# zhangzhousuper/Radish_PT

Measured on AMD Instinct MI355X. Metric: Mrays/s, higher is better.
Workload: dtype f32

## Files before the change

### radish_pt_amd/api.py

```python
import ctypes as C
import os

import numpy as np

from . import hostlib
from . import layouts as L

_HERE = os.path.dirname(os.path.abspath(__file__))
HIP_LIB_PATH = os.environ.get("RADISH_HIP_LIB") or os.path.join(_HERE, "csrc", "libradish_hip.so")

RDH_PT_MEGAKERNEL, RDH_PT_WAVEFRONT, RDH_PT_SORT_MATERIAL, RDH_PT_COUNT, RDH_PT_PROFILE = 0, 1, 2, 4, 8
RDH_PT_PERSISTENT = 16
RDH_PT_NO_SCHEDULE = 32
RDH_PT_ONE_LANE_PER_PIXEL = 64
RDH_PT_MEGA_GBUFFER = RDH_PT_ONE_LANE_PER_PIXEL
RDH_PT_NO_DEFER = 128
RDH_PT_WG_PER_RAY = 256
RDH_PT_PARTITION_GBUFFER = 512
RDH_PT_RESTIR_FUSED = 1024
RDH_PT_WF_SUBFRAMES = 2048
RDH_PT_WF_SMALL_LISTS = 4096
RDH_PT_NO_PAIRS = 16384
RDH_PT_NO_PACKETS = 8192
RDH_PT_PAIRS = 32768
# ... 595 lines not shown
        self.rank, self.world = rank, world

    def comm_destroy(self):
        self.check(lib().rdh_comm_destroy(self.h))

    @staticmethod
    def comm_init_all(ctxs):
        n = len(ctxs)
        arr = (C.c_void_p * n)(*[c.h for c in ctxs])
        rc = lib().rdh_comm_init_all(arr, n)
        if rc != 0:
            ctxs[0].check(rc)
        for i, c in enumerate(ctxs):
            c.rank, c.world = i, n

    @staticmethod
    def path_trace_gathered_all(ctxs, direct_frames, indirect_frames, iter, looper, max_depth, flags=RDH_PT_PERSISTENT):
        n = len(ctxs)
        arr = (C.c_void_p * n)(*[c.h for c in ctxs])
        px = ctxs[0].width * ctxs[0].height * 3
        d = (C.c_void_p * n)(*[c._ptr(t, px, "path_trace_gathered_all: direct") for c, t in zip(ctxs, direct_frames)])
        i = (C.c_void_p * n)(*[c._ptr(t, px, "path_trace_gathered_all: indirect") for c, t in zip(ctxs, indirect_frames)])
        rc = lib().rdh_path_trace_gathered_all(arr, n, d, i, iter, looper, max_depth, flags)
        if rc != 0:
            msgs = [lib().rdh_last_error(c.h) for c in ctxs]
            raise RadishError(f"libradish_hip error {rc}: " + "; ".join(f"ctx {k}: {m.decode()}" for k, m in enumerate(msgs) if m))

    def allgather_tiles(self, packed, frame):
        shard = self.tiles_per_rank() * self.tile * self.tile * 3
        self.check(lib().rdh_allgather_tiles(self.h, self._ptr(packed, shard, "allgather_tiles: packed"),
                                             self._ptr(frame, self.width * self.height * 3, "allgather_tiles: frame")))

    def path_trace_gathered(self, direct_frame, indirect_frame, iter, looper, max_depth, flags=RDH_PT_PERSISTENT):
        n = self.width * self.height * 3
        self.check(lib().rdh_path_trace_gathered(self.h, self._ptr(direct_frame, n, "path_trace_gathered: direct"),
                                                 self._ptr(indirect_frame, n, "path_trace_gathered: indirect"), iter, looper,
                                                 max_depth, flags))

    def restir_exchange(self):
        self.check(lib().rdh_restir_exchange(self.h))

    def comm_set_overlap(self, enable):
        self.check(lib().rdh_comm_set_overlap(self.h, 1 if enable else 0))

    def comm_join(self):
        self.check(lib().rdh_comm_join(self.h))

    @staticmethod
    def _all_error(ctxs, rc):
        msgs = [lib().rdh_last_error(c.h) for c in ctxs]
        raise RadishError(f"libradish_hip error {rc}: " + "; ".join(f"ctx {k}: {m.decode()}" for k, m in enumerate(msgs) if m))

    @staticmethod
    def gbuffer_exchange_all(ctxs, gb_cs):
        n = len(ctxs)
        arr = (C.c_void_p * n)(*[c.h for c in ctxs])
        gbs = (GBufferC * n)(*gb_cs)
        rc = lib().rdh_gbuffer_exchange_all(arr, n, gbs)
        if rc != 0:
            Context._all_error(ctxs, rc)

    @staticmethod
    def restir_direct_gathered_all(ctxs, direct_frames, iter, looper, gb_cs, reuse_mask, ris_count=32, num_spatial=5, temporal_clamp=20,
                                   faithful_ris=1, flags=0):
        n = len(ctxs)
        arr = (C.c_void_p * n)(*[c.h for c in ctxs])
        px = ctxs[0].width * ctxs[0].height * 3
        d = (C.c_void_p * n)(*[c._ptr(t, px, "restir_direct_gathered_all") for c, t in zip(ctxs, direct_frames)])
        gbs = (GBufferC * n)(*gb_cs)
        p = RestirParamsC(reuse_mask, ris_count, num_spatial, temporal_clamp, faithful_ris)
        rc = lib().rdh_restir_direct_gathered_all(arr, n, d, iter, looper, gbs, C.byref(p), flags)
        if rc != 0:
            Context._all_error(ctxs, rc)

    def restir_direct_gathered(self, direct_frame, iter, looper, gb_c, reuse_mask, ris_count=32, num_spatial=5, temporal_clamp=20,
                               faithful_ris=1, flags=0):
        p = RestirParamsC(reuse_mask, ris_count, num_spatial, temporal_clamp, faithful_ris)
        self.check(lib().rdh_restir_direct_gathered(self.h, self._ptr(direct_frame, self.width * self.height * 3, "restir_direct_gathered"),
                                                    iter, looper, C.byref(gb_c), C.byref(p), flags))

    def gbuffer_exchange(self, gb_c):
        self.check(lib().rdh_gbuffer_exchange(self.h, C.byref(gb_c)))

    def restir_read(self, which):
        out = np.zeros(self.width * self.height, dtype=L.RESERVOIR_DTYPE)
        self.check(lib().rdh_restir_read(self.h, which, out.ctypes.data))
        return out

    def restir_read_scratch(self, which):
        nbytes = int(lib().rdh_restir_read_scratch(self.h, which, None, 0))
        if nbytes < 0:
            self.check(nbytes)
        out = np.zeros(nbytes // 4, np.int32 if which == 2 else np.float32)
        got = int(lib().rdh_restir_read_scratch(self.h, which, out.ctypes.data, nbytes))
        if got < 0:
            self.check(got)
        return out if which == 2 else out.reshape(-1, 6)

    def trace_closest(self, rays, hits, flags=RDH_PT_PERSISTENT):
        n = rays.numel() // 6
        self.check(lib().rdh_trace_closest(self.h, self._ptr(rays, 6 * n, "trace_closest: rays"), n,
                                           self._ptr(hits, 4 * n, "trace_closest: hits", _torch().int32), flags))

    def trace_occluded(self, segments, out, flags=RDH_PT_PERSISTENT):
        n = segments.numel() // 6
        self.check(lib().rdh_trace_occluded(self.h, self._ptr(segments, 6 * n, "trace_occluded: segments"), n,
                                            self._ptr(out, n, "trace_occluded: out", _torch().int32), flags))

    def dump_rays(self, looper, max_depth):
        torch = _torch()
        nc, na = C.c_int64(0), C.c_int64(0)
        self.check(lib().rdh_dump_rays(self.h, looper, max_depth, None, 0, None, 0, C.byref(nc), C.byref(na)))
        dev = torch.device("cuda", self.device)
        closest = torch.zeros(max(nc.value, 1), 6, device=dev)
        segs = torch.zeros(max(na.value, 1), 6, device=dev)
        n2, a2 = C.c_int64(0), C.c_int64(0)
        self.check(lib().rdh_dump_rays(self.h, looper, max_depth, closest.data_ptr(), nc.value, segs.data_ptr(), na.value,
                                       C.byref(n2), C.byref(a2)))
        assert (n2.value, a2.value) == (nc.value, na.value)
        return closest[:nc.value], segs[:na.value]

    def set_occupancy_share(self, share):
        self.check(lib().rdh_set_occupancy_share(self.h, share))

    def counters_reset(self):
        self.check(lib().rdh_counters_reset(self.h))

    def counters(self):
        c = CountersC()
        self.check(lib().rdh_counters_read(self.h, C.byref(c)))
        return c.as_dict()

    def synchronize(self):
        self.check(lib().rdh_synchronize(self.h))

    def profile_reset(self):
        self.check(lib().rdh_profile_reset(self.h))

    def profile_read(self):
        ms, n = C.c_double(0), C.c_int64(0)
        self.check(lib().rdh_profile_read(self.h, C.byref(ms), C.byref(n)))
        return ms.value, n.value

    def debug_persist_stamps(self):
        out = np.zeros((5, 4096), dtype=np.uint64)
        self.check(lib().rdh_debug_persist_stamps(self.h, out.ctypes.data))
        return out

    def debug_wf_stamps(self):
        fn = lib().rdh_debug_wf_stamps
        fn.argtypes, fn.restype = [C.c_void_p, C.c_void_p, C.c_int64, C.POINTER(C.c_int32), C.POINTER(C.c_int32)], C.c_int32
        stages, waves = C.c_int32(0), C.c_int32(0)
        self.check(fn(self.h, None, 0, C.byref(stages), C.byref(waves)))
        out = np.zeros((stages.value, waves.value, 3), dtype=np.uint64)
        self.check(fn(self.h, out.ctypes.data, out.size, C.byref(stages), C.byref(waves)))
        return out

    def debug_persist_phases(self):
        out = np.zeros(16, dtype=np.uint64)
        self.check(lib().rdh_debug_persist_phases(self.h, out.ctypes.data))
        return out

    def last_kernel_ms(self):
        ms = C.c_float(0)
        self.check(lib().rdh_last_kernel_ms(self.h, C.byref(ms)))
        return ms.value


class ReservoirReuse:
    NONE, Temporal, Spatial, TemporalSpatial = 0, 1, 2, 3


class Settings:
    traceDepth = 0
    useReservoir = True
    reservoirReuse = ReservoirReuse.Temporal
    accumulate = False
    ptFlags = RDH_PT_PERSISTENT
    restirNumSpatial = 5
    restirRISCount = 32
    restirTemporalClamp = 20
    restirFaithfulRIS = 1


class State:
    camChanged = True
    looper = 0
    scene = None


class DevScene:

    def __init__(self):
        self.ctx = None

    def create(self, scene_data, device=0):
        self.ctx = Context(device)
        self.ctx.upload_scene(scene_data)

    def destroy(self):
        if self.ctx:
            self.ctx.close()
            self.ctx = None


class Scene:

    def __init__(self, scene_data, camera, device=0):
        self.data = scene_data
        self.camera = camera
        self.devScene = DevScene()
        self.devScene.create(scene_data, device)

    def clear(self):
        self.devScene.destroy()


def _ctx():
    if State.scene is None or State.scene.devScene.ctx is None:
        raise RadishError("State.scene is not set")
    ctx = State.scene.devScene.ctx
    ctx.set_camera(State.scene.camera)
    return ctx


def _advance_looper():
    State.looper = (State.looper + 1) % SOBOL_SAMPLE_NUM


def pathTraceInit():
    _ctx().synchronize()


def pathTraceFree():
    pass


def pathTrace(directIllum, indirectIllum, iter):
    ctx = _ctx()
    ctx.path_trace(directIllum, indirectIllum, iter, State.looper, Settings.traceDepth, Settings.ptFlags)
    ctx.synchronize()
    _advance_looper()


def pathTraceSamples(directIllum, indirectIllum, iter, samples):
    ctx = _ctx()
    ctx.path_trace_samples(directIllum, indirectIllum, iter, State.looper, samples, Settings.traceDepth, Settings.ptFlags)
    ctx.synchronize()
    State.looper = (State.looper + samples) % SOBOL_SAMPLE_NUM


def pathTraceDirect(directIllum, iter):
    ctx = _ctx()
    ctx.path_trace_direct(directIllum, iter, State.looper, Settings.ptFlags & RDH_PT_COUNT)
    ctx.synchronize()
    _advance_looper()


class ToneMapping:
    NONE, Filmic, ACES = 0, 1, 2


def copyImageToPBO(devPBO, devImage, width, height, toneMapping=ToneMapping.NONE, scale=1.0):
    torch = _torch()
    n = width * height
    if devImage.dtype == torch.int32:
        kind = 3
    elif devImage.dtype == torch.float32:
        kind = {3 * n: 0, 2 * n: 1, n: 2}.get(devImage.numel())
    else:
        kind = None
    if kind is None or devPBO.numel() * devPBO.element_size() != 4 * n:
        raise RadishError("copyImageToPBO: image/PBO shape does not match width*height")
    _ctx().copy_image_to_pbo(devPBO, devImage, width, height, kind, toneMapping, scale)


def ReSTIRInit():
    _ctx().restir_init()


def ReSTIRFree():
    if State.scene is not None and State.scene.devScene.ctx is not None:
        State.scene.devScene.ctx.restir_free()


def ReSTIRDirect(directIllum, iter, gBuffer):
    ctx = _ctx()
    ctx.restir_direct(directIllum, iter, State.looper, gBuffer.c_struct(), Settings.reservoirReuse,
                      Settings.restirRISCount, Settings.restirNumSpatial, Settings.restirTemporalClamp,
                      Settings.restirFaithfulRIS, Settings.ptFlags & RDH_PT_COUNT)
    ctx.synchronize()
    _advance_looper()


class GBuffer:

    def __init__(self):
        self.width = self.height = 0
        self.frameIdx = 0
        self.lastCam = None

    def create(self, width, height, device=0):
        torch = _torch()
        n = width * height
        dev = torch.device("cuda", device)
        self.width, self.height = width, height
        self.albedo = torch.zeros(n, 3, dtype=torch.float32, device=dev)
# ... 135 lines not shown
```

### radish_pt_amd/csrc/device/kernels_wave.h

```cpp
#pragma once
#include "kernels_pt.h"
#include "wg_trace.h"

namespace rd {

constexpr int kWfLitCap = 8192;
constexpr int kWfLitShadow = 0x40000000;
constexpr int kMaxWaveDepth = 32;

struct alignas(128) WaveCounter {
    int v;
    int pad[31];
};
#ifndef RD_WF_TICKET_SHARDS
#define RD_WF_TICKET_SHARDS 8
#endif
constexpr int kTicketShards = RD_WF_TICKET_SHARDS;
struct WaveCounters {
    WaveCounter rayCount[kMaxWaveDepth + 2];
    WaveCounter shadowCount[kMaxWaveDepth + 2];
    WaveCounter litCount[kMaxWaveDepth + 2];
    WaveCounter traceHead[kMaxWaveDepth + 2];
    WaveCounter shadeHead[kMaxWaveDepth + 2][4];
    WaveCounter traceTicket[kMaxWaveDepth + 2][kTicketShards];
    WaveCounter shadeTicket[kMaxWaveDepth + 2][kTicketShards];
};

struct WaveWorkspace {
    float4 *ro[2];
    float4 *rd[2];
    float4 *thr[2];
    float4 *prevPos[2];
    float4 *accD;
    float4 *accI;
    float4 *nee[2];
    float4 *sht[2];
    uint2 *rng[2];
    int4 *hit;
    int *rayq[2];
    int *shadowq;
    int *litq[2];
    int litCap;
    int *treeOvf;
    int treeOvfDepth;
#ifdef RD_WF_STAMPS
    unsigned long long *stamps;
    int stampWaves;
#endif
    WaveCounters *ctr;
};

constexpr unsigned kWfNeeNone = 2u;
RD_DEV float wfNeeTag(int home, unsigned kind) { return __uint_as_float(((unsigned)home << 2) | kind); }
RD_DEV void wfAddNee(const WaveWorkspace &w, float4 n) {
    const unsigned tag = __float_as_uint(n.w), kind = tag & 3u;
    if (kind == kWfNeeNone) return;
    float4 *acc = (kind == 0u ? w.accD : w.accI) + (tag >> 2);
    const float4 a = *acc;
    *acc = make_float4(a.x + n.x, a.y + n.y, a.z + n.z, 0.f);
}

RD_DEV Ray wfSlotRay(const WaveWorkspace &w, int set, int p, bool shadow, float &limit) {
    if (shadow) {
        const float4 x = w.prevPos[set][p], y = w.sht[set][p];
        return shadowRay(mk3(x.x, x.y, x.z), mk3(y.x, y.y, y.z), limit);
    }
    const float4 o = w.ro[set][p], d = w.rd[set][p];
    limit = 3.402823466e+38f;
    return Ray{mk3(o.x, o.y, o.z), mk3(d.x, d.y, d.z)};
}

struct WaveSlotPath {
    const WaveWorkspace &w;
    const int rs, p;
    const int wr, q;
    int home;
    const bool delta;
    RD_DEV v3 throughput() {
        const float4 t = w.thr[rs][p];
        home = __float_as_int(t.w);
        return mk3(t.x, t.y, t.z);
    }
    RD_DEV float samplePdf() const { return w.ro[rs][p].w; }
    RD_DEV bool sampleDelta() const { return delta; }
    RD_DEV v3 prevPos() const { const float4 c = w.prevPos[rs][p]; return mk3(c.x, c.y, c.z); }
    RD_DEV void setDirect(v3 v) { w.accD[home] = make_float4(v.x, v.y, v.z, 0.f); }
    RD_DEV void addIndirect(v3 v) { const float4 a = w.accI[home]; w.accI[home] = make_float4(a.x + v.x, a.y + v.y, a.z + v.z, 0.f); }
    RD_DEV Sampler rng(const DScene &s) const { const uint2 r = w.rng[rs][p]; return Sampler{s.sobol, r.x, (int)r.y}; }
    RD_DEV void setNee(v3 c, float nw) { w.nee[wr][q] = make_float4(c.x, c.y, c.z, wfNeeTag(home, nw < 0.f ? kWfNeeNone : (nw == 0.f ? 0u : 1u))); }
    RD_DEV void setPrevPos(v3 x) { w.prevPos[wr][q] = make_float4(x.x, x.y, x.z, 0.f); }
    RD_DEV void setRay(const Ray &ray, float pdf, bool deltaSample, v3 throughput, const Sampler &rng) {
        w.ro[wr][q] = make_float4(ray.o.x, ray.o.y, ray.o.z, pdf);
        w.rd[wr][q] = make_float4(ray.d.x, ray.d.y, ray.d.z, deltaSample ? 1.f : 0.f);
        w.thr[wr][q] = make_float4(throughput.x, throughput.y, throughput.z, __int_as_float(home));
        w.rng[wr][q] = make_uint2(rng.scramble, (unsigned)rng.ptr);
    }
};


RD_DEV void waveAppend(bool pred, int item, int *queue, int *count) {
    unsigned long long mask = __ballot(pred);
    if (mask == 0ull) return;
    int leader = __ffsll((long long)mask) - 1;
    int base = 0;
    if ((int)(threadIdx.x & 63u) == leader) base = atomicAdd(count, __popcll(mask));
    base = __shfl(base, leader, 64);
    if (pred) queue[base + __popcll(mask & laneMaskLt())] = item;
}

constexpr int kShadeChunks = 4;
constexpr int kShadePacket = 64 * kShadeChunks;
RD_DEV void waveAppendN(const bool (&pred)[kShadeChunks], const int (&item)[kShadeChunks], int *queue, int *count) {
    unsigned long long m[kShadeChunks];
    int total = 0;
#pragma unroll
    for (int j = 0; j < kShadeChunks; j++) {
        m[j] = __ballot(pred[j]);
        total += __popcll(m[j]);
    }
    if (total == 0) return;
    int base = 0;
    if ((threadIdx.x & 63u) == 0u) base = atomicAdd(count, total);
    base = __shfl(base, 0, 64);
#pragma unroll
    for (int j = 0; j < kShadeChunks; j++) {
        if (pred[j]) queue[base + __popcll(m[j] & laneMaskLt())] = item[j];
        base += __popcll(m[j]);
    }
}

constexpr int kPacket = 128;
RD_DEV int gridWaves() { return int(gridDim.x * (blockDim.x >> 6)); }
RD_DEV int workgroupTicket(WaveCounter *tickets) {
    __shared__ int ticket;
    if (threadIdx.x == 0) {
        const unsigned x = blockIdx.x % (unsigned)kTicketShards;
        ticket = int(x + (unsigned)kTicketShards * (unsigned)atomicAdd(&tickets[x].v, 1));
    }
    __syncthreads();
    return __builtin_amdgcn_readfirstlane(ticket);
}
RD_DEV int logicalWave(int wg) { return __builtin_amdgcn_readfirstlane(int(wg * int(blockDim.x >> 6) + int(threadIdx.x >> 6))); }
RD_DEV int wavePull(int *head, int packet = kPacket) {
    int base = 0;
    if ((threadIdx.x & 63u) == 0u) base = atomicAdd(head, packet);
    return __shfl(base, 0, 64) + gridWaves() * packet;
}

RD_DEV unsigned subFrameBlocks(const PixelMap &pm, int part, int parts) { return (unsigned)(pm.numBlocks - part + parts - 1) / (unsigned)parts; }
constexpr int kSobolRows = 10000;
__global__ __launch_bounds__(256) void k_wf_raygen(DScene s, DCamera cam, PixelMap pm, WaveWorkspace w, int looper, int samples, int part,
                                                   int parts) {
    unsigned wg;
    const unsigned nLocal = subFrameBlocks(pm, part, parts);
    const unsigned nGroups = nLocal * (unsigned)samples;
    bool wgValid = xcdSwizzle(blockIdx.x, (nGroups + 3u) >> 2, wg);
    unsigned lane = threadIdx.x & 63u;
    unsigned group = wgValid ? wg * 4u + (threadIdx.x >> 6) : 0xffffffffu / 64u;
    const bool inRange = wgValid && group < nGroups;
    const unsigned b = group / nLocal, blockLocal = group - b * nLocal;
    Pix px = mapPixel(pm, inRange ? blockLocal * (unsigned)parts + (unsigned)part : 0xffffffffu / 64u, lane);
    bool valid = px.valid && inRange;
    int p = int(group * 64u + lane);
    bool listed = false;
    if (valid) {
        Sampler rng = makeSeededRandomEngine(int(((unsigned)looper + b) % (unsigned)kSobolRows), px.index, 0, s.sobol);
        Ray ray = cameraSample(cam, px.x, px.y, sample4D(rng));
        w.ro[0][p] = make_float4(ray.o.x, ray.o.y, ray.o.z, 0.f);
        w.rd[0][p] = make_float4(ray.d.x, ray.d.y, ray.d.z, 0.f);
        w.accD[p] = make_float4(0.f, 0.f, 0.f, 0.f);
        w.accI[p] = make_float4(0.f, 0.f, 0.f, 0.f);
        w.rng[0][p] = make_uint2(rng.scramble, (unsigned)rng.ptr);
        if (fabs_(ray.d.x) < 1.1e-6f || fabs_(ray.d.y) < 1.1e-6f || fabs_(ray.d.z) < 1.1e-6f) {
            const int at = atomicAdd(&w.ctr->litCount[0].v, 1);
            if (at < w.litCap) {
                w.litq[0][at] = p;
                listed = true;
            }
        }
    }
    if (inRange) w.rayq[0][p] = valid ? (listed ? -2 - p : p) : -1;
    if (blockIdx.x == 0 && threadIdx.x == 0) w.ctr->rayCount[0].v = int(nGroups) * 64;
}

#ifndef RD_REFILL_MIN
#define RD_REFILL_MIN 16
#endif
#ifndef RD_WF_FINISH_MIN
#define RD_WF_FINISH_MIN 16
#endif
#ifndef RD_WF_SHADOW_FIRST
#define RD_WF_SHADOW_FIRST 0
#endif
constexpr int kWfStampKinds = 3;
#ifdef RD_WF_STAMPS
#define RD_WF_STAMP(kind) do { if (stampAt && (threadIdx.x & 63u) == 0u) stampAt[kind] = wall_clock64(); } while (0)
#define RD_WF_STAMP_DRY() do { if (exhausted && !stampedDry) { stampedDry = true; RD_WF_STAMP(1); } } while (0)
#else
#define RD_WF_STAMP(kind) ((void)0)
#define RD_WF_STAMP_DRY() ((void)0)
#endif
#ifndef RD_WF_COOP_LONE
#define RD_WF_COOP_LONE 1
#endif

#ifndef RD_WF_TRACE_WAVES
#define RD_WF_TRACE_WAVES 7
#endif
#ifndef RD_WF_PAIR_WAVES
#define RD_WF_PAIR_WAVES 1
#endif
template <bool COUNT, bool PAIRS = false>
__global__ __launch_bounds__(256, PAIRS && !COUNT ? RD_WF_PAIR_WAVES : (!COUNT ? RD_WF_TRACE_WAVES : 1)) void k_wf_trace(DScene s, WaveWorkspace w, int k) {
    WaveCounters *c = w.ctr;
    const int wg = workgroupTicket(c->traceTicket[k]);
#ifdef RD_WF_STAMPS
    unsigned long long *const stampAt = w.stamps ? w.stamps + ((size_t)k * (size_t)w.stampWaves + (size_t)logicalWave(wg)) * kWfStampKinds : nullptr;
    bool stampedDry = false;
    RD_WF_STAMP(0);
#endif
    const int nShadow = (k > 0) ? c->shadowCount[k - 1].v : 0;
    const int nRay = c->rayCount[k].v;
    const int total = nShadow + nRay;
    const int *rayq = w.rayq[k & 1];
    const int set = k & 1;
    WalkStats ws{0, 0};
    unsigned nClosest = 0, nAny = 0, nHits = 0;
    const int end = s.bvhSize;
    const int END = end;

    int resNext = logicalWave(wg) * kPacket, resEnd = resNext + kPacket;
    bool exhausted = resNext >= total;
    if (resEnd > total) resEnd = total;
    RD_WF_STAMP_DRY();

    bool alive = false;
    bool isShadow = false;
    int p = -1;
    RaySlab rs;
    rs.o = rs.d = rs.inv = mk3(0.f);
    rs.cls = 0;
    const NodeRec *nodes = s.nodes[0];
    int ord = 0, cur = kPairNone;
    PairStack sp{0, 0};
    int node = END, pending = -1;
    float tmax = 0.f;
    int hitPrim = -1;
    v2 hitBary = mk2(0.f, 0.f);
    bool occluded = false;

    constexpr int kStackEntries = PAIRS ? 4 * kPairLds * 64 : 1;
    __shared__ union WfTraceLds {
        WgTraceSharedT<256> wg;
        int2 stack[kStackEntries];
    } lds;
    WgTraceSharedT<256> &wgsh = lds.wg;
    int2 *const stk = lds.stack + (PAIRS ? int(threadIdx.x >> 6) * kPairLds * 64 : 0);
    int2 *const ovf = PAIRS ? reinterpret_cast<int2 *>(w.treeOvf) + (size_t)logicalWave(wg) * (size_t)w.treeOvfDepth * 64 : nullptr;
    const int nLit = c->litCount[k].v < w.litCap ? c->litCount[k].v : w.litCap;
    for (int it = wg; it < nLit; it += int(gridDim.x)) {
        const int e = w.litq[k & 1][it];
        const bool sh = (e & kWfLitShadow) != 0;
        const int pp = e & (kWfLitShadow - 1);
        float lim;
        const Ray ray = wfSlotRay(w, set, pp, sh, lim);
        const RaySlab urs = makeRaySlab(ray);
        if (urs.cls == 0 || end == 0) continue;
        const NodeRec *un = s.nodes[getMTBVHId(-ray.d)];
        const CoopTrace ct = sh ? wgTraceWhole<true, 256>(s, un, urs, lim, wgsh) : wgTraceWhole<false, 256>(s, un, urs, lim, wgsh);
        if (threadIdx.x == 0) {
            if (sh) {
                nAny++;
                if (!ct.found) wfAddNee(w, w.nee[set][pp]);
            } else {
                nClosest++;
                const bool hit = ct.hitPrim != -1;
                if (hit) nHits++;
                w.hit[pp] = make_int4(ct.hitPrim, __float_as_int(hit ? ct.bary.x : 0.f), __float_as_int(hit ? ct.bary.y : 0.f),
                                      hit ? int(s.primClass[ct.hitPrim]) : 0);
            }
            if (COUNT) {
                ws.nodes += ct.nodes;
                ws.tris += ct.tris;
            }
        }
    }
    if (PAIRS) __syncthreads();
    bool firstRound = true;
    bool fromList = false;
    for (;;) {
        bool doStart = false;
        fromList = false;
        if (firstRound) {
            firstRound = false;
            const int it = wg + (int(threadIdx.x & 63u) * 4 + int(threadIdx.x >> 6)) * int(gridDim.x);
            if (it < nLit) {
                const int e = w.litq[k & 1][it];
                doStart = true;
                fromList = true;
                isShadow = (e & kWfLitShadow) != 0;
                p = e & (kWfLitShadow - 1);
            }
        }
        unsigned long long idle = __ballot(!alive && !doStart && p < 0);
        int nIdle = __popcll(idle);
        if (!exhausted && nIdle >= RD_REFILL_MIN) {
            int myRank = __popcll(idle & laneMaskLt());
            int taken = 0;
            while (taken < nIdle && !exhausted) {
                if (resNext == resEnd) {
                    resNext = wavePull(&c->traceHead[k].v);
                    resEnd = resNext + kPacket;
                    if (resNext >= total) {
                        exhausted = true;
                        break;
                    }
                    if (resEnd > total) resEnd = total;
                }
                int avail = resEnd - resNext;
                int give = (nIdle - taken) < avail ? (nIdle - taken) : avail;
                if (!alive && !doStart && p < 0 && myRank >= taken && myRank < taken + give) {
                    const int item = resNext + (myRank - taken);
                    doStart = true;
#if RD_WF_SHADOW_FIRST
                    isShadow = item < nShadow;
                    p = isShadow ? w.shadowq[item] : rayq[item - nShadow];
#else
                    isShadow = item >= nRay;
                    p = isShadow ? w.shadowq[item - nRay] : rayq[item];
#endif
                }
                resNext += give;
                taken += give;
            }
        }
        RD_WF_STAMP_DRY();
        if (doStart) {
            if (p >= 0) {
                const Ray ray = wfSlotRay(w, set, p, isShadow, tmax);
                if (isShadow) nAny++;
                else nClosest++;
                rs = makeRaySlab(ray);
                pending = -1;
                if (PAIRS) {
                    ord = getMTBVHId(-ray.d);
                    sp = PairStack{0, 0};
                    if (rs.cls == 0 || end == 0) pairStart<COUNT>(s, rs, tmax, cur, pending, ws);
                    else cur = kPairFresh;
                    alive = true;
                } else {
                    nodes = s.nodes[getMTBVHId(-ray.d)];
                    node = 0;
                    alive = node != END;
                }
                hitPrim = -1;
                occluded = false;
                if (fromList && rs.cls != 0 && end != 0) {
                    if (isShadow) nAny--;
                    else nClosest--;
                    alive = false;
                    p = -1;
                }
            }
        }
        unsigned long long am = __ballot(alive);
        if (am == 0ull) {
            if (exhausted) break;
            continue;
        }

        {
            unsigned long long lit = __ballot(PAIRS ? (alive && cur == kPairFresh) : (alive && rs.cls != 0 && node == 0 && pending < 0));
            while (lit) {
                const int L = __ffsll((long long)lit) - 1;
                lit &= lit - 1ull;
                const bool shadowL = readlaneI(isShadow ? 1 : 0, L) != 0;
                const NodeRec *un = PAIRS ? s.nodes[0] + (size_t)readlaneI(ord, L) * (size_t)(end + 1) : readlanePtr(nodes, L);
                const RaySlab ur = readlaneRay(rs, L);
                const float lim = readlaneF(tmax, L);
                CoopTrace ct = shadowL ? coopTraceWhole<true>(s, un, ur, lim) : coopTraceWhole<false>(s, un, ur, lim);
                if (int(threadIdx.x & 63u) == L) {
                    hitPrim = ct.hitPrim;
                    hitBary = ct.bary;
                    tmax = ct.tmax;
                    occluded = ct.found;
                    node = END;
                    cur = kPairNone;
                    alive = false;
                    if (COUNT) {
                        ws.nodes += ct.nodes;
                        ws.tris += ct.tris;
                    }
                }
            }
        }
        if (PAIRS) {
            bool busy = alive && pending < 0;
            const int nStart = __popcll(__ballot(busy));
            if (nStart > 0) {
                const int minWalk = (nStart * (RD_LEAF_DEN - RD_LEAF_NUM) + RD_LEAF_DEN - 1) / RD_LEAF_DEN;
                const int lane = int(threadIdx.x & 63u);
                do {
                    pairPopOne<COUNT>(stk, lane, ovf, tmax, busy, cur, sp, pending, ws);
                    if (busy && cur >= 0) {
                        pairStep<COUNT>(s.pairs, stk, lane, ovf, rs, tmax, ord, cur, sp, pending, ws);
                        busy = pending < 0 && (cur >= 0 || sp.sp > 0);
                    }
                } while (__popcll(__ballot(busy)) >= (minWalk > 1 ? minWalk : 1));
                alive = alive && (pending >= 0 || cur >= 0 || sp.sp > 0);
            }
        } else
        {
            bool walking = alive && pending < 0;
            const int nStart = __popcll(__ballot(walking));
#if RD_WF_COOP_LONE
            if (nStart == 1) {
                const int L = __ffsll((long long)__ballot(walking)) - 1;
                CoopResult cr = coopWalk(readlanePtr(nodes, L), readlaneI(node, L), end, readlaneRay(rs, L), readlaneF(tmax, L), RD_COOP_WINDOWS);
                if (int(threadIdx.x & 63u) == L) {
                    node = cr.node;
                    pending = cr.pending;
                    if (COUNT) ws.nodes += cr.visited;
                    alive = (node != end) || pending >= 0;
                }
            } else
#endif
            if (nStart > 0) {
                const int minWalk = (nStart * (RD_LEAF_DEN - RD_LEAF_NUM) + RD_LEAF_DEN - 1) / RD_LEAF_DEN;
                do {
                    if (walking) {
                        if (COUNT) ws.nodes++;
                        float4 lo = nodes[node].lo_prim;
                        float4 hi = nodes[node].hi_next;
                        float boundDist;
                        bool boundHit = aabbFast(lo, hi, rs, boundDist);
                        if (boundHit && boundDist < tmax) {
                            pending = __float_as_int(lo.w);
                            node++;
                        } else {
                            node = __float_as_int(hi.w);
                        }
                        walking = pending < 0 && node != END;
                        alive = (node != END) || pending >= 0;
                    }
                } while (__popcll(__ballot(walking)) >= (minWalk > 1 ? minWalk : 1));
            }
        }
        if (alive && pending >= 0) {
            TriVerts t = loadTri(s.tris, pending);
            float dist;
            v2 bary;
            if (COUNT) ws.tris++;
            bool hit = intersectTriangle(rs, t.a, t.b, t.c, bary, dist);
            if (hit && dist < tmax) {
                if (isShadow) {
                    occluded = true;
                    node = END;
                    cur = kPairNone;
                    sp = PairStack{0, 0};
                } else {
                    hitPrim = pending;
                    tmax = dist;
                    hitBary = bary;
                }
// ... 177 lines not shown
```

### radish_pt_amd/csrc/radish_hip.hip

```cpp
#include "radish_hip.h"

#include <hip/hip_runtime.h>
#include <dlfcn.h>

#include <algorithm>
#include <cfloat>
#include <climits>
#include <cmath>
#include <cstdarg>
#include <cstdio>
#include <cstring>
#include <mutex>
#include <string>
#include <type_traits>
#include <utility>
#include <vector>

#include "device/kernels_pt.h"
#include "device/kernels_restir.h"
#include "device/kernels_wave.h"
#include "device/kernels_persist.h"
#include "device/kernels_walk.h"
#include "device/kernels_display.h"
#include "device/kernels_denoise.h"
// ... 522 lines not shown
    pm.world = c->world;
    pm.tilesPerRank = (pm.numTiles + pm.world - 1) / pm.world;
    pm.packed = (c->world > 1 || c->forcePacked) ? 1 : 0;
    int bpe = pm.tile / 8;
    pm.numBlocks = pm.tilesPerRank * bpe * bpe;
    return pm;
}

constexpr int kPairMinNodes = 0;
bool usePairs(const rdh_ctx *c, uint32_t flags) {
    if (!c->scene.ds.pairs || (flags & RDH_PT_NO_PAIRS)) return false;
    if (flags & RDH_PT_PAIRS) return true;
    if (c->pairMode >= 0) return c->pairMode != 0;
    return c->scene.ds.bvhSize >= kPairMinNodes;
}

bool usePackets(uint32_t flags) {
    static const int env = getenv("RADISH_PACKETS") ? atoi(getenv("RADISH_PACKETS")) : 1;
    return env != 0 && !(flags & RDH_PT_NO_PACKETS);
}

unsigned gridFor(const PixelMap &pm) {
    unsigned work = (unsigned)(pm.numBlocks + 3) / 4;
    return ((work + 7u) / 8u) * 8u;
}

unsigned gridBlocks(const PixelMap &pm) { return (((unsigned)pm.numBlocks + 7u) / 8u) * 8u; }

int settleTree(rdh_ctx *c) {
    if (!c->scene.treePending) return RDH_OK;
    HIP_TRY(c, hipEventSynchronize(c->evTree));
    c->scene.treePending = false;
    if (c->scene.treeRefit) {
        c->scene.treeRefit = false;
        if (!c->scene.ds.pairs) return RDH_OK;
        const int4 lo = c->hTreeHdr.as<int4>()[1], hi = c->hTreeHdr.as<int4>()[2];
        c->scene.ds.rootLo = make_float4(__builtin_bit_cast(float, lo.x), __builtin_bit_cast(float, lo.y), __builtin_bit_cast(float, lo.z), c->scene.ds.rootLo.w);
        c->scene.ds.rootHi = make_float4(__builtin_bit_cast(float, hi.x), __builtin_bit_cast(float, hi.y), __builtin_bit_cast(float, hi.z), c->scene.ds.rootHi.w);
        return RDH_OK;
    }
    const int4 *hdr = c->hTreeHdr.as<int4>(), h0 = hdr[0], lo = hdr[1], hi = hdr[2];
    if (h0.y != 0) {
        c->scene.haveScene = false;
        return fail(c, RDH_ERR_STATE, "device BVH build failed (error bits %d); the scene must be uploaded again", h0.y);
    }
    constexpr int kMaxPairDepth = 2048;
    const PairRec *pairs = c->scene.updPairs ? c->scene.updPairs : c->scene.ds.pairs;
    if (h0.x <= kMaxPairDepth) {
        c->scene.ds.pairs = pairs;
        c->scene.ds.treeDepth = h0.x;
        c->scene.ds.rootLo = make_float4(__builtin_bit_cast(float, lo.x), __builtin_bit_cast(float, lo.y), __builtin_bit_cast(float, lo.z),
                                   __builtin_bit_cast(float, lo.w));
        c->scene.ds.rootHi = make_float4(__builtin_bit_cast(float, hi.x), __builtin_bit_cast(float, hi.y), __builtin_bit_cast(float, hi.z),
                                   __builtin_bit_cast(float, hi.w));
    } else {
        c->scene.ds.pairs = nullptr;
        c->scene.ds.treeDepth = 0;
    }
    return RDH_OK;
}

int settleLights(rdh_ctx *c) {
    if (!c->scene.lightsPending) return RDH_OK;
    HIP_TRY(c, hipEventSynchronize(c->evLights));
    c->scene.lightsPending = false;
    c->scene.ds.sumLightPowerInv = c->hLightSums.as<float>()[1];
    return RDH_OK;
}

int requireReady(rdh_ctx *c) {
    if (!c) return RDH_ERR_ARGS;
    if (c->scene.haveScene) {
        int rc = settleTree(c);
        if (rc) return rc;
        if ((rc = settleLights(c))) return rc;
    }
    if (!c->scene.haveScene) return fail(c, RDH_ERR_NO_SCENE, "no scene uploaded (rdh_scene_upload)");
    if (!c->haveCamera) return fail(c, RDH_ERR_NO_SCENE, "no camera set (rdh_set_camera)");
    return RDH_OK;
}

constexpr size_t kProfilePairs = 8192;

long profBegin(rdh_ctx *c, uint32_t flags) {
    if (!(flags & RDH_PT_PROFILE) || c->profUsed >= kProfilePairs) return -1;
    if (c->profEvents.size() < 2 * (c->profUsed + 1)) {
        hipEvent_t a = nullptr, b = nullptr;
        if (newEvent(c, &a, true) || newEvent(c, &b, true)) return -1;
        c->profEvents.push_back(a);
        c->profEvents.push_back(b);
    }
    long i = (long)c->profUsed++;
    hipEventRecord(c->profEvents[2 * i], c->stream);
    return i;
}
void profEnd(rdh_ctx *c, long i) {
    if (i >= 0) hipEventRecord(c->profEvents[2 * i + 1], c->stream);
}

constexpr unsigned kPersistentGrid = 256u * 8u;

template <typename T>
int wfAlloc(rdh_ctx *c, T **out, size_t count) {
    void *p = nullptr;
    HIP_TRY(c, hipMalloc(&p, std::max<size_t>(count * sizeof(T), 16)));
    c->wfAllocs.push_back(p);
    *out = static_cast<T *>(p);
    return RDH_OK;
}

int wavefrontEnsure(rdh_ctx *c, const PixelMap &pm, int samples) {
    long long slots = (long long)pm.numBlocks * 64 * samples;
    if (c->wfCapacity >= slots) return RDH_OK;
    for (void *p : c->wfAllocs) hipFree(p);
    c->wfAllocs.clear();
    c->wfCapacity = 0;
    const size_t n0 = (size_t)slots, n1 = (size_t)((slots / 64 + 1) / 2) * 64;
    for (int h = 0; h < kWfParts; h++) {
        WaveWorkspace &w = c->wf[h];
        const size_t n = h == 0 ? n0 : n1;
        int rc = RDH_OK;
        for (int set = 0; set < 2 && rc == RDH_OK; set++) {
            if ((rc = wfAlloc(c, &w.ro[set], n)) || (rc = wfAlloc(c, &w.rd[set], n)) || (rc = wfAlloc(c, &w.thr[set], n)) ||
                (rc = wfAlloc(c, &w.prevPos[set], n)) || (rc = wfAlloc(c, &w.nee[set], n)) || (rc = wfAlloc(c, &w.sht[set], n)) ||
                (rc = wfAlloc(c, &w.rng[set], n)))
                return rc;
        }
        if ((rc = wfAlloc(c, &w.accD, n)) || (rc = wfAlloc(c, &w.accI, n)) ||
            (rc = wfAlloc(c, &w.hit, n)) || (rc = wfAlloc(c, &w.rayq[0], n)) || (rc = wfAlloc(c, &w.rayq[1], n)) ||
            (rc = wfAlloc(c, &w.shadowq, n)) || (rc = wfAlloc(c, &w.ctr, 1)) || (rc = wfAlloc(c, &w.litq[0], (size_t)kWfLitCap)) ||
            (rc = wfAlloc(c, &w.litq[1], (size_t)kWfLitCap)))
            return rc;
        w.litCap = 0;
    }
    if (!c->evWfFork) {
        int rc;
        if ((rc = newEvent(c, &c->evWfFork)) || (rc = newEvent(c, &c->evWfJoin))) return rc;
        HIP_TRY(c, hipStreamCreateWithFlags(&c->wfStream, hipStreamNonBlocking));
        if ((rc = newEvent(c, &c->evWfJoin3))) return rc;
    }
    c->wfCapacity = slots;
    return RDH_OK;
}

int wavefrontPathTrace(rdh_ctx *c, const PixelMap &pm, float *d_direct, float *d_indirect, int iter, int looper, int samples,
                       int maxDepth, uint32_t flags) {
    if (maxDepth > kMaxWaveDepth) return fail(c, RDH_ERR_ARGS, "maxDepth %d exceeds %d", maxDepth, kMaxWaveDepth);
    const bool count = (flags & RDH_PT_COUNT) != 0, sort = (flags & RDH_PT_SORT_MATERIAL) != 0;
    const bool tree = usePairs(c, flags);
    unsigned traceRes = 0, shadeRes = 0;
    int rq = RDH_OK;
    withBools([&](auto cnt, auto pr) { rq = residentGrid(c, k_wf_trace<cnt.value, pr.value>, 256, &traceRes); }, count, tree);
    if (rq || (rq = residentGrid(c, k_wf_shade, 256, &shadeRes))) return rq;
    const unsigned traceGrid = sharedGrid(c, std::min(traceRes, kPersistentGrid), kUnbounded);
    const unsigned shadeGrid = sharedGrid(c, std::min(shadeRes, kPersistentGrid), kUnbounded);
    static const int partsEnv = getenv("RADISH_WF_PARTS") ? atoi(getenv("RADISH_WF_PARTS")) : kWfPartsDefault;
    int parts = ((flags & RDH_PT_WF_SUBFRAMES) && pm.numBlocks >= 2048) ? (partsEnv >= 1 && partsEnv <= kWfParts ? partsEnv : kWfPartsDefault) : 1;
    const int ovfDepth = c->scene.ds.treeDepth + 1;
    const size_t ovfNeed = (size_t)traceGrid * 4 * 64 * (size_t)ovfDepth * 2;
    if (tree && parts > 1 && (size_t)parts * ovfNeed * sizeof(int) > kWfStripBudget) parts = 1;
    hipStream_t sts[kWfParts] = {c->stream, c->sideStream, c->wfStream};
    if (tree) {
        for (int h = 0; h < parts; h++) {
            if (int rc = grow(c, c->wfTreeOvf[h], ovfNeed, ovfNeed * sizeof(int), Busy::Device)) return rc;
            c->wf[h].treeOvf = c->wfTreeOvf[h].as<int>();
            c->wf[h].treeOvfDepth = ovfDepth;
        }
    }
#ifdef RD_WF_STAMPS
    {
        const size_t stamps = (size_t)(maxDepth + 1) * traceGrid * 4 * kWfStampKinds;
        if (int rc = grow(c, c->wfStamps, stamps, stamps * sizeof(unsigned long long), Busy::Device)) return rc;
        HIP_TRY(c, hipMemsetAsync(c->wfStamps.p, 0, stamps * sizeof(unsigned long long), c->stream));
        for (int h = 0; h < kWfParts; h++) {
            c->wf[h].stamps = h == 0 ? c->wfStamps.as<unsigned long long>() : nullptr;
            c->wf[h].stampWaves = (int)(traceGrid * 4);
        }
        c->wfStampStages = maxDepth + 1;
        c->wfStampWaves = (int)(traceGrid * 4);
    }
#endif
    const long pf = parts >= 2 ? profBegin(c, flags) : -1;
    if (parts >= 2) {
        HIP_TRY(c, hipEventRecord(c->evWfFork, c->stream));
        for (int h = 1; h < parts; h++) HIP_TRY(c, hipStreamWaitEvent(sts[h], c->evWfFork, 0));
    }
    int rc = RDH_OK;
    auto keep = [&](hipError_t e, const char *what) {
        if (e != hipSuccess && rc == RDH_OK) rc = fail(c, (int)e, "HIP error (%s:%d): %s: %s", __FILE__, __LINE__, what, hipGetErrorString(e));
    };
    for (int h = 0; h < parts; h++) {
        const unsigned waves = traceGrid * 4u;
        c->wf[h].litCap = (int)(waves * 64u < (unsigned)kWfLitCap ? waves * 64u : (unsigned)kWfLitCap);
        if (flags & RDH_PT_WF_SMALL_LISTS) c->wf[h].litCap = 4;
    }
    for (int h = 0; h < parts; h++) {
        hipStream_t st = sts[h];
        WaveWorkspace &w = c->wf[h];
        const unsigned nLocal = (unsigned)(pm.numBlocks - h + parts - 1) / (unsigned)parts;
        const unsigned gridBlk = (((nLocal * (unsigned)samples + 3u) / 4u + 7u) / 8u) * 8u;
        keep(hipMemsetAsync(w.ctr, 0, sizeof(WaveCounters), st), "hipMemsetAsync(wavefront counters)");
        hipLaunchKernelGGL(k_wf_raygen, dim3(gridBlk), dim3(256), 0, st, c->scene.ds, c->cam, pm, w, looper, samples, h, parts);
    }
    for (int k = 0; k <= maxDepth && rc == RDH_OK; k++) {
        for (int h = 0; h < parts; h++) {
            hipStream_t st = sts[h];
            WaveWorkspace &w = c->wf[h];
            long pe = (h == 0 && parts == 1) ? profBegin(c, flags) : -1;
            withBools([&](auto cnt, auto pr) {
                hipLaunchKernelGGL((k_wf_trace<cnt.value, pr.value>), dim3(traceGrid), dim3(256), 0, st, c->scene.ds, w, k);
            }, count, tree);
            profEnd(c, pe);
            hipLaunchKernelGGL(k_wf_shade, dim3(shadeGrid), dim3(256), 0, st, c->scene.ds, w, k, maxDepth, sort ? 1 : 0);
        }
        keep(hipGetLastError(), "wavefront stage launch");
    }
    for (int h = 0; h < parts && rc == RDH_OK; h++) {
        hipStream_t st = sts[h];
        const unsigned nLocal = (unsigned)(pm.numBlocks - h + parts - 1) / (unsigned)parts;
        const unsigned gridBlk = (((nLocal + 3u) / 4u + 7u) / 8u) * 8u;
        hipLaunchKernelGGL(k_wf_finish, dim3(gridBlk), dim3(256), 0, st, pm, c->wf[h], iter, samples, d_direct, d_indirect, h, parts);
    }
    keep(hipGetLastError(), "k_wf_finish");
    if (parts >= 2) {
        hipError_t e1 = hipEventRecord(c->evWfJoin, c->sideStream);
        hipError_t e2 = hipStreamWaitEvent(c->stream, c->evWfJoin, 0);
        hipError_t e3 = hipEventRecord(c->evWfJoin3, c->wfStream);
        hipError_t e4 = hipStreamWaitEvent(c->stream, c->evWfJoin3, 0);
        if (e1 != hipSuccess || e2 != hipSuccess || e3 != hipSuccess || e4 != hipSuccess) {
            hipStreamSynchronize(c->sideStream);
            hipStreamSynchronize(c->wfStream);
            keep(e1 != hipSuccess ? e1 : (e2 != hipSuccess ? e2 : (e3 != hipSuccess ? e3 : e4)), "wavefront join");
        }
    }
    profEnd(c, pf);
    return rc;
}

int ensureStackOverflow(rdh_ctx *c, unsigned resident) {
    const size_t ints = (size_t)resident * 64 * (size_t)(c->scene.ds.treeDepth + 1) * 2;
    return grow(c, c->treeOvf, ints, ints * sizeof(int), Busy::Device);
}

uint32_t resolveStructure(const rdh_ctx *c, const PixelMap &pm, uint32_t flags) {
    if (!(flags & RDH_PT_AUTO)) return flags;
    flags &= ~(RDH_PT_AUTO | RDH_PT_WAVEFRONT | RDH_PT_SORT_MATERIAL | RDH_PT_WF_SUBFRAMES | RDH_PT_PERSISTENT);
    const bool wavefront = c->scene.ds.bvhSize >= 100000 && pm.numBlocks >= 12000;
    return flags | (wavefront ? (RDH_PT_WAVEFRONT | RDH_PT_SORT_MATERIAL | RDH_PT_WF_SUBFRAMES) : RDH_PT_PERSISTENT);
}

int packetBudget(uint32_t flags) { return (flags & RDH_PT_WF_SMALL_LISTS) ? 4 : kPacketBudget; }

int launchWalk(rdh_ctx *c, const float *d_rays, long long n, int4 *d_hits, int *d_occ, bool count, const int *deferCount = nullptr,
               const int *deferList = nullptr, int slotList = 0, bool pairs = false, bool packets = false, int budget = kPacketBudget) {
    const bool any = d_occ != nullptr, defer = deferCount != nullptr;
    packets = packets && !any && n > 0 && (n + 255) / 256 <= 0x7fffffffll;
    if (pairs && !c->scene.ds.pairs) return fail(c, RDH_ERR_UNSUPPORTED, "RDH_PT_PAIRS: the uploaded node arrays are not six orderings of one binary tree, or that tree is more than 2 048 levels deep");
    unsigned resGrid = 0;
    int rc = RDH_OK;
    withBools([&](auto a) {
        rc = pairs ? residentGrid(c, k_walk_pair<false, a.value>, 64, &resGrid) : residentGrid(c, k_walk_persistent<false, a.value>, 64, &resGrid);
    }, any);
    if (rc) return rc;
    const unsigned grid = sharedGrid(c, resGrid, (unsigned long long)((n + 63) / 64));
    const int ovfDepth = c->scene.ds.treeDepth + 1;
    if (pairs && !packets && (rc = ensureStackOverflow(c, resGrid))) return rc;
    int2 *const ovf = c->treeOvf.as<int2>();
    if (!packets) HIP_TRY(c, hipMemsetAsync(c->dPersist, 0, offsetof(PersistCounters, deferred), c->stream));
    if (defer) {
        if ((rc = forkLiteral(c))) return rc;
        withBools([&](auto cnt, auto a) {
            hipLaunchKernelGGL((k_trace_wg_list<cnt.value, a.value>), dim3(kWalkDeferCap), dim3(kWgTraceThreads), 0, c->litStream, c->scene.ds, d_rays, deferList, deferCount, d_hits, d_occ);
        }, count, any);
    }
    if (packets) {
        const unsigned pgrid = (unsigned)((n + 255) / 256);
        withBools([&](auto cnt, auto def) {
            hipLaunchKernelGGL((k_walk_packet<cnt.value, def.value>), dim3(pgrid), dim3(256), 0, c->stream, c->scene.ds, d_rays, n, d_hits, deferCount, slotList, budget);
        }, count, defer);
    } else {
        withBools([&](auto cnt, auto a, auto def) {
            if (pairs)
                hipLaunchKernelGGL((k_walk_pair<cnt.value, a.value, def.value>), dim3(grid), dim3(64), 0, c->stream, c->scene.ds, d_rays, n, d_hits, d_occ,
                                   c->dPersist, ovf, ovfDepth, deferCount, slotList);
            else
                hipLaunchKernelGGL((k_walk_persistent<cnt.value, a.value, def.value>), dim3(grid), dim3(64), 0, c->stream, c->scene.ds, d_rays, n, d_hits, d_occ,
                                   c->dPersist, deferCount, slotList);
        }, count, any, defer);
    }
    if (defer) joinLiteral(c);
    HIP_TRY(c, hipGetLastError());
    return RDH_OK;
}

RestirSplit splitLayout(Carver &k, size_t slots) {
    RestirSplit sp;
    sp.st = k.take<float4>(slots * 48);
    sp.hits = k.take<int4>(slots * 16);
    sp.rays = k.take<float>(slots * 24);
    sp.segs = k.take<float>(slots * 24);
    sp.rawResv = k.take<float>(slots * 36);
    sp.occ = k.take<int>(slots * 4);
    sp.deferCount = k.take<int>(16 + 2 * sizeof(int) * kRestirDeferCap);
    sp.deferList = sp.deferCount + 4;
    return sp;
}

void timeBegin(rdh_ctx *c) {
    hipEventRecord(c->evStart, c->stream);
}
int timeEnd(rdh_ctx *c, const char *what) {
    hipEventRecord(c->evStop, c->stream);
    c->timed = true;
    hipError_t e = hipGetLastError();
    if (e != hipSuccess) return fail(c, (int)e, "HIP error: %s: %s", what, hipGetErrorString(e));
    return RDH_OK;
}

}

extern "C" {

int rdh_create(rdh_ctx **out, int device) {
    if (!out) return RDH_ERR_ARGS;
    *out = nullptr;
    int n = 0;
    if (hipGetDeviceCount(&n) != hipSuccess || n <= 0 || device < 0 || device >= n) return RDH_ERR_NO_DEVICE;
    if (hipSetDevice(device) != hipSuccess) return RDH_ERR_NO_DEVICE;
    rdh_ctx *c = new rdh_ctx;
// ... 2416 lines not shown
```

Baseline: 3009.

## Dedicate workgroups to lit-list rays and cap pair-trace occupancy

Workgroups whose ticket falls below the lit-list count now handle only the special lit rays and take no initial packet. The remaining workgroups get the static initial packets, and the dynamic head is offset past them. The pair-trace kernel gains an explicit waves-per-EU maximum, and the host caps the trace grid to CUs times that maximum. Extra stamp instrumentation is added for debugging. The intent is to stop lit-ray work from delaying packet tracing and to reduce oversubscription, at the risk of idle duty groups or lower occupancy.

```diff
diff --git a/radish_pt_amd/api.py b/radish_pt_amd/api.py
--- a/radish_pt_amd/api.py
+++ b/radish_pt_amd/api.py
@@ -771,7 +771,7 @@
         fn.argtypes, fn.restype = [C.c_void_p, C.c_void_p, C.c_int64, C.POINTER(C.c_int32), C.POINTER(C.c_int32)], C.c_int32
         stages, waves = C.c_int32(0), C.c_int32(0)
         self.check(fn(self.h, None, 0, C.byref(stages), C.byref(waves)))
-        out = np.zeros((stages.value, waves.value, 3), dtype=np.uint64)
+        out = np.zeros((stages.value, waves.value, 6), dtype=np.uint64)
         self.check(fn(self.h, out.ctypes.data, out.size, C.byref(stages), C.byref(waves)))
         return out
 
diff --git a/radish_pt_amd/csrc/device/kernels_wave.h b/radish_pt_amd/csrc/device/kernels_wave.h
--- a/radish_pt_amd/csrc/device/kernels_wave.h
+++ b/radish_pt_amd/csrc/device/kernels_wave.h
@@ -46,6 +46,7 @@
 #ifdef RD_WF_STAMPS
     unsigned long long *stamps;
     int stampWaves;
+    int stampStages;
 #endif
     WaveCounters *ctr;
 };
@@ -141,10 +142,15 @@
     return __builtin_amdgcn_readfirstlane(ticket);
 }
 RD_DEV int logicalWave(int wg) { return __builtin_amdgcn_readfirstlane(int(wg * int(blockDim.x >> 6) + int(threadIdx.x >> 6))); }
-RD_DEV int wavePull(int *head, int packet = kPacket) {
+RD_DEV int wavePull(int *head, int packet) {
     int base = 0;
     if ((threadIdx.x & 63u) == 0u) base = atomicAdd(head, packet);
     return __shfl(base, 0, 64) + gridWaves() * packet;
+}
+RD_DEV int tracePull(int *head, int headBase) {
+    int base = 0;
+    if ((threadIdx.x & 63u) == 0u) base = atomicAdd(head, kPacket);
+    return __builtin_amdgcn_readlane(base, 0) + headBase;
 }
 
 RD_DEV unsigned subFrameBlocks(const PixelMap &pm, int part, int parts) { return (unsigned)(pm.numBlocks - part + parts - 1) / (unsigned)parts; }
@@ -183,6 +189,9 @@
     if (blockIdx.x == 0 && threadIdx.x == 0) w.ctr->rayCount[0].v = int(nGroups) * 64;
 }
 
+#ifndef RD_WF_DUTY_SHARE
+#define RD_WF_DUTY_SHARE 0
+#endif
 #ifndef RD_REFILL_MIN
 #define RD_REFILL_MIN 16
 #endif
@@ -192,13 +201,16 @@
 #ifndef RD_WF_SHADOW_FIRST
 #define RD_WF_SHADOW_FIRST 0
 #endif
-constexpr int kWfStampKinds = 3;
+constexpr int kWfStampKinds = 6;
 #ifdef RD_WF_STAMPS
 #define RD_WF_STAMP(kind) do { if (stampAt && (threadIdx.x & 63u) == 0u) stampAt[kind] = wall_clock64(); } while (0)
-#define RD_WF_STAMP_DRY() do { if (exhausted && !stampedDry) { stampedDry = true; RD_WF_STAMP(1); } } while (0)
+#define RD_WF_STAMP_DRY() do { if (exhausted && !stampedDry) { stampedDry = true; RD_WF_STAMP(1); if (stampAt && (threadIdx.x & 63u) == 0u) *headDry = 1ull; } } while (0)
+#define RD_WF_STAMP_HELD(held) do { if (stampAt && !stampedHeld && *headDry != 0ull) { \
+        stampedHeld = true; const int h_ = (held); if ((threadIdx.x & 63u) == 0u) stampAt[4] = 1ull + (unsigned long long)h_; } } while (0)
 #else
 #define RD_WF_STAMP(kind) ((void)0)
 #define RD_WF_STAMP_DRY() ((void)0)
+#define RD_WF_STAMP_HELD(held) ((void)0)
 #endif
 #ifndef RD_WF_COOP_LONE
 #define RD_WF_COOP_LONE 1
@@ -210,13 +222,18 @@
 #ifndef RD_WF_PAIR_WAVES
 #define RD_WF_PAIR_WAVES 1
 #endif
+#ifndef RD_WF_PAIR_MAX_WAVES
+#define RD_WF_PAIR_MAX_WAVES 6
+#endif
 template <bool COUNT, bool PAIRS = false>
-__global__ __launch_bounds__(256, PAIRS && !COUNT ? RD_WF_PAIR_WAVES : (!COUNT ? RD_WF_TRACE_WAVES : 1)) void k_wf_trace(DScene s, WaveWorkspace w, int k) {
+__global__ __launch_bounds__(256) __attribute__((amdgpu_waves_per_eu(PAIRS && !COUNT ? RD_WF_PAIR_WAVES : (!COUNT ? RD_WF_TRACE_WAVES : 1),
+                                                                      PAIRS && !COUNT ? RD_WF_PAIR_MAX_WAVES : 8))) void k_wf_trace(DScene s, WaveWorkspace w, int k) {
     WaveCounters *c = w.ctr;
     const int wg = workgroupTicket(c->traceTicket[k]);
 #ifdef RD_WF_STAMPS
     unsigned long long *const stampAt = w.stamps ? w.stamps + ((size_t)k * (size_t)w.stampWaves + (size_t)logicalWave(wg)) * kWfStampKinds : nullptr;
-    bool stampedDry = false;
+    volatile unsigned long long *const headDry = w.stamps ? w.stamps + (size_t)w.stampStages * (size_t)w.stampWaves * kWfStampKinds + k : nullptr;
+    bool stampedDry = false, stampedHeld = false;
     RD_WF_STAMP(0);
 #endif
     const int nShadow = (k > 0) ? c->shadowCount[k - 1].v : 0;
@@ -229,7 +246,11 @@
     const int end = s.bvhSize;
     const int END = end;
 
-    int resNext = logicalWave(wg) * kPacket, resEnd = resNext + kPacket;
+    const int nLit = c->litCount[k].v < w.litCap ? c->litCount[k].v : w.litCap;
+    const int dutyGroups = RD_WF_DUTY_SHARE ? 0 : (nLit < int(gridDim.x) ? nLit : int(gridDim.x));
+    const bool duty = wg < dutyGroups;
+    const int headBase = (int(gridDim.x) - dutyGroups) * int(blockDim.x >> 6) * kPacket;
+    int resNext = duty ? headBase : (logicalWave(wg) - dutyGroups * int(blockDim.x >> 6)) * kPacket, resEnd = duty ? resNext : resNext + kPacket;
     bool exhausted = resNext >= total;
     if (resEnd > total) resEnd = total;
     RD_WF_STAMP_DRY();
@@ -257,7 +278,6 @@
     WgTraceSharedT<256> &wgsh = lds.wg;
     int2 *const stk = lds.stack + (PAIRS ? int(threadIdx.x >> 6) * kPairLds * 64 : 0);
     int2 *const ovf = PAIRS ? reinterpret_cast<int2 *>(w.treeOvf) + (size_t)logicalWave(wg) * (size_t)w.treeOvfDepth * 64 : nullptr;
-    const int nLit = c->litCount[k].v < w.litCap ? c->litCount[k].v : w.litCap;
     for (int it = wg; it < nLit; it += int(gridDim.x)) {
         const int e = w.litq[k & 1][it];
         const bool sh = (e & kWfLitShadow) != 0;
@@ -285,6 +305,10 @@
             }
         }
     }
+    RD_WF_STAMP(3);
+#ifdef RD_WF_STAMPS
+    if (stampAt && (threadIdx.x & 63u) == 0u) stampAt[5] = 1ull + (unsigned long long)nLit;
+#endif
     if (PAIRS) __syncthreads();
     bool firstRound = true;
     bool fromList = false;
@@ -305,11 +329,12 @@
         unsigned long long idle = __ballot(!alive && !doStart && p < 0);
         int nIdle = __popcll(idle);
         if (!exhausted && nIdle >= RD_REFILL_MIN) {
+            RD_WF_STAMP_HELD(resEnd - resNext);
             int myRank = __popcll(idle & laneMaskLt());
             int taken = 0;
             while (taken < nIdle && !exhausted) {
                 if (resNext == resEnd) {
-                    resNext = wavePull(&c->traceHead[k].v);
+                    resNext = tracePull(&c->traceHead[k].v, headBase);
                     resEnd = resNext + kPacket;
                     if (resNext >= total) {
                         exhausted = true;
diff --git a/radish_pt_amd/csrc/radish_hip.hip b/radish_pt_amd/csrc/radish_hip.hip
--- a/radish_pt_amd/csrc/radish_hip.hip
+++ b/radish_pt_amd/csrc/radish_hip.hip
@@ -698,6 +698,11 @@
     int rq = RDH_OK;
     withBools([&](auto cnt, auto pr) { rq = residentGrid(c, k_wf_trace<cnt.value, pr.value>, 256, &traceRes); }, count, tree);
     if (rq || (rq = residentGrid(c, k_wf_shade, 256, &shadeRes))) return rq;
+    if (tree && !count) {
+        int cus = 0;
+        if (int rc = cuCount(c, &cus)) return rc;
+        traceRes = std::min(traceRes, (unsigned)cus * (unsigned)RD_WF_PAIR_MAX_WAVES);
+    }
     const unsigned traceGrid = sharedGrid(c, std::min(traceRes, kPersistentGrid), kUnbounded);
     const unsigned shadeGrid = sharedGrid(c, std::min(shadeRes, kPersistentGrid), kUnbounded);
     static const int partsEnv = getenv("RADISH_WF_PARTS") ? atoi(getenv("RADISH_WF_PARTS")) : kWfPartsDefault;
@@ -715,12 +720,13 @@
     }
 #ifdef RD_WF_STAMPS
     {
-        const size_t stamps = (size_t)(maxDepth + 1) * traceGrid * 4 * kWfStampKinds;
+        const size_t stamps = (size_t)(maxDepth + 1) * traceGrid * 4 * kWfStampKinds + (size_t)(maxDepth + 1);
         if (int rc = grow(c, c->wfStamps, stamps, stamps * sizeof(unsigned long long), Busy::Device)) return rc;
         HIP_TRY(c, hipMemsetAsync(c->wfStamps.p, 0, stamps * sizeof(unsigned long long), c->stream));
         for (int h = 0; h < kWfParts; h++) {
             c->wf[h].stamps = h == 0 ? c->wfStamps.as<unsigned long long>() : nullptr;
             c->wf[h].stampWaves = (int)(traceGrid * 4);
+            c->wf[h].stampStages = maxDepth + 1;
         }
         c->wfStampStages = maxDepth + 1;
         c->wfStampWaves = (int)(traceGrid * 4);
```

Measured after the change: 3049 (median of 6 runs). +1.3%, better.
